# rgl-epfl/large-steps-pytorch

Measured on AMD Instinct MI355X. Metric: from_differential_solves_per_sec, higher is better.
Workload: dtype f32; 1 GPU; cfg4_plane1m: 1000x1000 plane, V=1000000, nnz(M)=6992002, M=I+50*L_uniform, u=M v, k=3, factor once (not timed), re-solve timed; method=nested-dissection, device=AMD Radeon Graphics

## Files before the change

### include/largesteps_hip.h

```cpp
#ifndef LARGESTEPS_HIP_H
#define LARGESTEPS_HIP_H

#include <stddef.h>
#include <stdint.h>

#ifdef __cplusplus
extern "C" {
#endif

#define LS_VERSION 110

#define LS_OK 0
#define LS_E_INVALID (-1)
#define LS_E_INDEX (-2)
#define LS_E_WORKSPACE (-3)
#define LS_E_OVERFLOW (-4)
#define LS_E_STATE (-5)
#define LS_E_NOT_CONVERGED (-6)

#define LS_LAPLACIAN_UNIFORM 0
#define LS_LAPLACIAN_COT 1

int ls_version(void);
const char* ls_last_error(void);
// ... 97 lines not shown
    const int64_t* h_nodes;
    const int32_t* h_perm;
    const int32_t* h_ppos;
    int64_t n_bnd;
    const int32_t* h_push_ptr;
    const int32_t* h_push_tgt;
    int64_t n_front;
    const float* d_finv;
    const float* d_wf;
    const float* d_wb;
    const float* d_u4;
    const float* d_d4;
    const float* d_tri;
    const int32_t* d_sp_ptr;
    const void* d_sp_ent;
    int64_t n_sp_ptr, n_sp_ent;
    int32_t shard_rank, shard_count;
    int32_t tier_waves;
} ls_direct_arrays;
int ls_direct_create(const ls_direct_arrays* arrays, int device, void* stream, ls_direct** out);
int ls_direct_pick_tree(int64_t V, int* leaf_size, int* arity);
int ls_direct_tier_lds_bytes(int levels, int arity, const int32_t* h_s, const int32_t* h_b, const int32_t* h_own_start, int tier_levels,
                             int sparse_leaves, int waves, size_t* h_bytes);
int ls_direct_factor(const int32_t* d_rowptr, const int32_t* d_col, const float* d_val, int64_t V, int64_t nnz,
                     const float* d_positions, int leaf_size, int arity, int tier_levels, int sparse_leaves, int shard_rank,
                     int shard_count, int device, void* stream, ls_direct** out);
typedef struct ls_direct_options {
    int32_t struct_bytes;
    int32_t leaf_size, arity, tier_levels, sparse_leaves, shard_rank, shard_count;
    int32_t ordering;
    int32_t tier_waves;
} ls_direct_options;
int ls_direct_options_default(ls_direct_options* opt);
int ls_direct_factor_ex(const int32_t* d_rowptr, const int32_t* d_col, const float* d_val, int64_t V, int64_t nnz,
                        const float* d_positions, const ls_direct_options* opt, int device, void* stream, ls_direct** out);
int ls_direct_factor_refactorable(const int32_t* d_rowptr, const int32_t* d_col, const float* d_val, int64_t V, int64_t nnz,
                                  const float* d_positions, const ls_direct_options* opt, int device, void* stream, ls_direct** out);
int ls_direct_refactor(ls_direct* d, const int32_t* d_rowptr, const int32_t* d_col, const float* d_val, int64_t V, int64_t nnz,
                       void* stream);
int ls_direct_refactorable(const ls_direct* d, int* h_yes, size_t* h_retained_device_bytes);
int ls_release_scratch(int device);
int ls_direct_shape(const ls_direct* d, int* h_levels, int* h_arity, int* h_tier_levels, int* h_tier_workgroups,
                    int64_t* h_words_up, int64_t* h_words_down, int64_t* h_n_bnd);
int ls_direct_level_words(const ls_direct* d, int cap, int64_t* h_up, int64_t* h_down);
int ls_direct_level_rows(const ls_direct* d, int cap, int64_t* h_rows, int64_t* h_bnd);
int ls_direct_level_index_bytes(const ls_direct* d, int cap, int64_t* h_up, int64_t* h_down);
int ls_direct_tier_balance(const ls_direct* d, double* h_words4);
int ls_direct_launch_profile(const ls_direct* d, int cap, int* h_n, double* h_ms, int64_t* h_words, int32_t* h_level_lo,
                             int32_t* h_level_hi, int32_t* h_sweep);
int ls_direct_plan_quality(const ls_direct* d, int* h_ordering, double* h_words_per_vertex, double* h_spread, double* h_words_other);
int ls_direct_factor_seconds(const ls_direct* d, double* h_s3);
int ls_csr_is_symmetric(const int32_t* d_rowptr, const int32_t* d_col, const float* d_val, int64_t V, int64_t nnz, float tol,
                        int* h_symmetric, int device, void* stream);
int ls_direct_destroy(ls_direct* d);
int ls_direct_solve(ls_direct* d, const float* b, float* x, int k, void* stream);
int ls_direct_solve_part(ls_direct* d, const float* b, float* x, int k, int part, float* exchange, void* stream);
int ls_direct_shard_info(const ls_direct* d, int* h_rank, int* h_count, int* h_cut_level, int64_t* h_exchange_floats_per_column,
                         unsigned char* h_owned_rows);
int ls_direct_exchange_region(ls_direct* d, int k, float** h_region, int64_t* h_floats);

typedef struct ls_dist ls_dist;
int ls_dist_unique_id(void* h_id128);
int ls_dist_create(const void* h_id128, int rank, int world, int device, ls_dist** out);
int ls_dist_destroy(ls_dist* c);
int ls_dist_allreduce_sum(ls_dist* c, float* d_buf, int64_t n, void* stream);
int ls_dist_info(const ls_dist* c, int* h_rank, int* h_world);
int ls_dist_direct_solve(ls_dist* c, ls_direct* d, const float* b, float* x, int k, void* stream);
int ls_direct_set(ls_direct* d, const char* name, int value);
int ls_direct_info(const ls_direct* d, int64_t* h_factor_entries, int* h_launches, double* h_ms3);

int ls_remove_duplicates_workspace_bytes(int64_t V, size_t* h_bytes);
int ls_remove_duplicates(const float* verts, int64_t V, const void* faces, int idx_bytes, int64_t F, float* unique_verts,
                         int64_t* inverse, int64_t* new_faces, int64_t* h_n_unique, void* workspace, size_t ws_bytes, int device,
                         void* stream);

int ls_csr_transpose_workspace_bytes(int64_t V, int64_t nnz, size_t* h_bytes);
int ls_csr_transpose(const int32_t* rowptr, const int32_t* col, const float* val, int64_t V, int64_t nnz, int32_t* t_rowptr,
                     int32_t* t_col, float* t_val, void* workspace, size_t ws_bytes, int device, void* stream);
int ls_corner_ranks_workspace_bytes(int64_t F, int64_t V, size_t* h_bytes);
int ls_corner_ranks(const void* faces, int idx_bytes, int64_t F, int64_t V, int32_t* vptr, int32_t* cpos, void* workspace,
                    size_t ws_bytes, int device, void* stream);

int ls_normals_workspace_bytes(int64_t F, int64_t V, size_t* h_bytes);
int ls_face_normals(const float* verts, const void* faces, int idx_bytes, int64_t F, int64_t V, float* fn, int device, void* stream);
int ls_face_normals_backward(const float* verts, const void* faces, int idx_bytes, int64_t F, int64_t V, const int32_t* vptr,
                             const int32_t* cpos, const float* g_fn, float* grad_verts, void* workspace, size_t ws_bytes,
                             int device, void* stream);
int ls_vertex_normals(const float* verts, const void* faces, int idx_bytes, int64_t F, int64_t V, const int32_t* vptr,
                      const int32_t* cpos, const float* fn, float* out, float* raw, float* norms, void* workspace,
                      size_t ws_bytes, int device, void* stream);
int ls_vertex_normals_backward(const float* verts, const void* faces, int idx_bytes, int64_t F, int64_t V, const int32_t* vptr,
// ... 189 lines not shown
```

### large-steps-pytorch_amd/csrc/direct.hip

```cpp
#include "common.h"
#include <vector>
#include <chrono>
#include <algorithm>
#include <atomic>
#include <string.h>
#include <memory>
#include <mutex>

namespace ls {

struct alignas(64) Tile {
    int store;
    int row0, s, b, own_start, bnd_off, front_off;
    int leaf;
    int pfront_off, cix;
    int forward;
    int arity;
    long long finv_off, w_off;
};

static_assert(sizeof(Tile) == 64, "Tile layout");
__device__ __forceinline__ Tile load_tile(const Tile* __restrict__ tiles, int idx) {
    const int lane = threadIdx.x & 63;
    const int w = lane < 16 ? reinterpret_cast<const int*>(tiles)[(size_t)idx * 16 + lane] : 0;
// ... 705 lines not shown
    const float *finv = nullptr, *wf = nullptr, *wb = nullptr;
    const float *u4 = nullptr, *d4 = nullptr;
    const float* tri = nullptr;
    const int* sp_ptr = nullptr;
    const SpEnt* sp_ent = nullptr;
    float* braw = nullptr;
    float *bp = nullptr, *slots = nullptr, *xb = nullptr;
    int upper_lo = 0;
    int tier_root = 0, tier_phases = 0, tier_wgs = 0, tier_region = 0, tier_vec = 0, tier_tri = 0, tier_waves = TIER_WAVES;
    TierItem* d_items = nullptr;
    int* pull = nullptr;
    int64_t pull_base = 0;
    TierWG* d_wgs = nullptr;
    hipEvent_t busy = nullptr;
    hipStream_t last_stream = nullptr;
    bool used = false;
    std::vector<std::pair<void*, size_t>> tables;
    ls::RefactorState* refac = nullptr;
    bool factored = true;
    int shard_rank = 0, shard_count = 1, cut = 0;
    int64_t exch_f0 = 0, exch_f1 = 0;
    std::vector<unsigned char> owned_rows;
    bool nt_levels = false, nt_tier = false, nt_rule[2] = {false, false};
    double factor_s[3] = {0, 0, 0};
    double plan_q[4] = {0, 0, 0, 0};
    std::vector<LevelPlan> plan;
    int64_t factor_entries = 0, words_up = 0, words_down = 0;
    int profile = 0;
    std::vector<hipEvent_t> ev;
    struct LaunchMeta { int lo, hi, sweep; };
    std::vector<hipEvent_t> lev;
    std::vector<LaunchMeta> lmeta;
    std::vector<double> launch_ms;
    std::vector<int64_t> lvl_up, lvl_down;
    std::vector<int64_t> lvl_rows, lvl_bnd;
    std::vector<int64_t> lvl_idx_up, lvl_idx_down;
    double tier_balance[4] = {0, 0, 0, 0};
    double prof_ms[3] = {0, 0, 0};
#ifdef LS_TIER_STAMPS
    long long* stamps = nullptr;
#endif
};

static int pick_nw(int len, int target) {
    int nw = 1;
    while (nw < 16 && len > nw * target) nw *= 2;
// ... 191 lines not shown
    memset(nd.data(), 0, nd.size() * sizeof(NodeD));
    const int root = levels - tier_levels;
    for (int lv = root; lv < levels; ++lv)
        for (int64_t i = level_off[lv]; i < level_off[lv + 1]; ++i) {
            NodeD& q = nd[(size_t)i];
            q.s = s[i]; q.b = b[i]; q.own_start = own_start[i];
            const bool sparse = sparse_leaves && lv == levels - 1 && q.s >= 1;
            q.flags = (lv + 1 >= levels ? NODE_LEAF : 0) | (sparse ? NODE_SPARSE : NODE_QUAD);
        }
    std::vector<TierItem> items;
    std::vector<TierWG> wgs;
    int vec = 0, tri = 0;
    const size_t region = plan_tier(nd, level_off, levels, arity, root, 0, level_off[root + 1] - level_off[root], items, wgs, vec, tri, waves);
    return region ? ((region + 3) & ~(size_t)3) * sizeof(float) * waves : 0;
}

bool direct_tier_fits(int levels, int arity, const int* s, const int* b, const int* own_start, int tier_levels, bool sparse_leaves, int waves) {
    if (tier_levels <= 0) return true;
    if (tier_levels > levels || tier_levels > TIER_MAX_H) return false;
    const size_t bytes = direct_tier_lds(levels, arity, s, b, own_start, tier_levels, sparse_leaves, waves);
    return bytes && bytes <= (size_t)(waves == TIER_WAVES_FULL ? TIER_LDS_FULL : TIER_LDS);
}

extern "C" int ls_direct_tier_lds_bytes(int levels, int arity, const int32_t* h_s, const int32_t* h_b, const int32_t* h_own_start, int tier_levels,
                                        int sparse_leaves, int waves, size_t* h_bytes) {
    LS_REQUIRE(h_s && h_b && h_own_start && h_bytes && levels >= 1 && levels <= 30 && (arity == 2 || arity == 4 || arity == 8) &&
               tier_levels >= 1 && tier_levels <= levels && tier_levels <= TIER_MAX_H && (waves == TIER_WAVES || waves == TIER_WAVES_WIDE || waves == TIER_WAVES_FULL),
               LS_E_INVALID, "ls_direct_tier_lds_bytes: bad argument (1 <= tier_levels <= min(levels, %d); waves 4, 8 or 16)", TIER_MAX_H);
    *h_bytes = direct_tier_lds(levels, arity, h_s, h_b, h_own_start, tier_levels, sparse_leaves != 0, waves);
    return LS_OK;
}

bool direct_tier_full16(int64_t V, int arity, int levels, int tier_levels, int shard_count, int tier_waves) {
    if (tier_waves == TIER_WAVES_FULL) return tier_levels >= 2;
    if (tier_waves == TIER_WAVES || tier_waves == TIER_WAVES_WIDE) return false;
    return shard_count <= 1 && arity == 4 && levels >= 8 && V >= 800000 && tier_levels == levels - 4 && tier_levels <= TIER_MAX_H;
}


namespace {
struct CreatePlan {
    int levels = 0, arity = 0, cut = 0;
    int64_t sub_lo = 0, sub_hi = 1;
    std::vector<int64_t> level_off;
    std::vector<NodeD> nd;
    std::vector<int> parent;
// ... 93 lines not shown
    if (T.cut > root) { set_error("ls_direct_create: %d ranks need a cut below the tier's root level (tree too small)", d->shard_count); return LS_E_INVALID; }
    const int64_t span = T.span(T.cut, root), q_lo = T.sub_lo * span, q_hi = T.sub_hi * span;
    size_t region = 0;
    auto take_if_fits = [&](int waves, int budget) {
        std::vector<TierItem> items;
        std::vector<TierWG> wgs;
        int vec = 0, tri = 0;
        const size_t r = plan_tier(T.nd, T.level_off, levels, T.arity, root, q_lo, q_hi, items, wgs, vec, tri, waves);
        if (!r || ((r + 3) & ~(size_t)3) * sizeof(float) * waves > (size_t)budget) return;
        T.items.swap(items); T.wgs.swap(wgs); d->tier_vec = vec; d->tier_tri = tri; region = r; d->tier_waves = waves;
    };
    if (H <= TIER_MAX_H && direct_tier_full16(d->V, T.arity, levels, H, d->shard_count, tier_waves > 0 ? tier_waves : env.tier_waves.value_or(0)))
        take_if_fits(TIER_WAVES_FULL, TIER_LDS_FULL);
    if (!region) {
        region = H <= TIER_MAX_H ? plan_tier(T.nd, T.level_off, levels, T.arity, root, q_lo, q_hi, T.items, T.wgs, d->tier_vec, d->tier_tri) : 0;
        if (!region || region * sizeof(float) * TIER_WAVES > TIER_LDS) {
            set_error("ls_direct_create: a tier of %d levels does not fit the kernel (LDS per wave: %zu floats)", H, region);
            return LS_E_WORKSPACE;
        }
        if (H >= 2 && (int)T.wgs.size() <= 768 && (tier_waves > 0 ? tier_waves : env.tier_waves.value_or(TIER_WAVES_WIDE)) == TIER_WAVES_WIDE)
            take_if_fits(TIER_WAVES_WIDE, TIER_LDS_WIDE);
    }
    d->tier_root = root; d->tier_phases = H; d->tier_wgs = (int)T.wgs.size(); d->tier_region = (int)((region + 3) & ~(size_t)3);
    d->pull_base = T.nd[T.level_off[root]].front_off;
    T.pull.assign((size_t)std::max<int64_t>(0, T.nd[T.level_off[levels - 1]].front_off - d->pull_base) * T.arity, -1);
    for (int lv = root + 1; lv < levels; ++lv)
        for (int64_t i = T.level_off[lv]; i < T.level_off[lv + 1]; ++i) {
            const NodeD& n = T.nd[i];
            for (int k = 0; k < n.b; ++k) T.pull[(size_t)(n.pfront_off - d->pull_base + h_ppos[n.bnd_off + k]) * T.arity + n.cix] = n.bnd_off + k;
        }
    return LS_OK;
}

size_t plan_level(CreatePlan& T, int lv, int long_up, const NdEnv& env, int kmax, LevelPlan& p) {
    std::vector<Tile>& tiles = T.tiles;
    int64_t a0 = T.level_off[lv], a1 = T.level_off[lv + 1];
    if (lv >= T.cut) { const int64_t span = T.span(T.cut, lv); a0 = T.level_off[lv] + T.sub_lo * span; a1 = T.level_off[lv] + T.sub_hi * span; }
    auto tile_of = [&](int64_t i, int r, int forward) {
        const NodeD& n = T.nd[i];
        Tile t;
        t.store = 0; t.row0 = r; t.s = n.s; t.b = n.b; t.own_start = n.own_start; t.bnd_off = n.bnd_off; t.front_off = n.front_off;
        t.leaf = lv + 1 >= T.levels; t.pfront_off = n.pfront_off; t.cix = n.cix;
        t.forward = forward; t.arity = T.arity; t.finv_off = n.finv_off; t.w_off = n.w_off;
        return t;
    };
    int red_up = 0, red_down = 0;
// ... 266 lines not shown
    if (d->busy) (void)hipEventDestroy(d->busy);
    if (!d->tables.empty()) (void)hipDeviceSynchronize();
    for (const auto& t : d->tables)
        if (!ls::pool_give(d->device, t.first, t.second)) (void)hipFree(t.first);
    ls::refactor_state_free(d->refac);
    for (hipEvent_t e : d->ev) (void)hipEventDestroy(e);
#ifdef LS_TIER_STAMPS
    if (d->stamps) (void)hipFree(d->stamps);
#endif
    for (hipEvent_t e : d->lev) (void)hipEventDestroy(e);
    delete d;
    return LS_OK;
}

template <int K>
static int direct_solve_k(ls_direct* d, const float* b, float* x, hipStream_t st, int part, float* exchange) {
    const int top = d->tier_root - 1;
    TierArgs ta;
    ta.items = d->d_items; ta.wgs = d->d_wgs; ta.perm = d->perm; ta.mask = d->mask; ta.ppos = d->ppos;
    ta.pull = d->pull ? d->pull - (size_t)d->pull_base * d->arity : nullptr; ta.push_ptr = d->push_ptr; ta.push_tgt = d->push_tgt; ta.u4 = d->u4; ta.d4 = d->d4; ta.tri = d->tri;
    ta.sp_ptr = d->sp_ptr; ta.sp_ent = d->sp_ent; ta.bprime = d->bp; ta.braw = d->braw; ta.slots = d->slots; ta.xb = d->xb;
    ta.arity = d->arity; ta.phases = d->tier_phases; ta.region_floats = d->tier_region; ta.vec_floats = d->tier_vec;
    ta.upper_lo = d->upper_lo; ta.upper_hi = (int)d->V;
#ifdef LS_TIER_STAMPS
    const size_t stamp_n = (size_t)d->tier_wgs * d->tier_waves * TIER_STAMP_SLOTS;
    if (d->profile == 2 && !d->stamps && stamp_n) LS_HIP(hipMalloc((void**)&d->stamps, 2 * stamp_n * sizeof(long long)));
    if (d->profile == 2 && d->stamps) LS_HIP(hipMemsetAsync(d->stamps, 0, 2 * stamp_n * sizeof(long long), st));
    ta.stamps = d->profile == 2 ? d->stamps : nullptr;
#endif
    const size_t tier_lds = (size_t)d->tier_region * d->tier_waves * sizeof(float);
    const bool nt_tier = d->nt_tier && d->tier_waves != TIER_WAVES_WIDE, nt = d->nt_levels;
    int n_mark = 0;
    auto mark = [&](int lo, int hi, int sweep) -> hipError_t {
        if (d->profile != 3) return hipSuccess;
        while ((int)d->lev.size() <= n_mark + 1) { hipEvent_t e; const hipError_t r = hipEventCreate(&e); if (r != hipSuccess) return r; d->lev.push_back(e); }
        if ((int)d->lmeta.size() <= n_mark) d->lmeta.resize((size_t)n_mark + 1);
        d->lmeta[(size_t)n_mark] = {lo, hi, sweep};
        return hipEventRecord(d->lev[(size_t)n_mark++], st);
    };
    auto mark_end = [&]() -> hipError_t {
        if (d->profile != 3) return hipSuccess;
        hipError_t r = hipEventRecord(d->lev[(size_t)n_mark], st);
        if (r == hipSuccess) r = hipStreamSynchronize(st);
        d->launch_ms.assign((size_t)n_mark, 0.0);
        d->lmeta.resize((size_t)n_mark);
        for (int i = 0; i < n_mark && r == hipSuccess; ++i) { float ms = 0; r = hipEventElapsedTime(&ms, d->lev[(size_t)i], d->lev[(size_t)i + 1]); d->launch_ms[(size_t)i] = ms; }
        return r;
    };
    const size_t exch_off = (size_t)d->exch_f0 * d->arity * K, exch_n = (size_t)(d->exch_f1 - d->exch_f0) * d->arity * K;
    if (part != 1) {
    if (d->profile) LS_HIP(hipEventRecord(d->ev[0], st));
    if (part == 0 && exch_n) LS_HIP(hipMemsetAsync(d->slots + exch_off, 0, exch_n * sizeof(float), st));
    if (d->tier_wgs) {
// ... 139 lines not shown
    if (h_cut_level) *h_cut_level = d->cut;
    if (h_exchange_floats_per_column) *h_exchange_floats_per_column = (d->exch_f1 - d->exch_f0) * d->arity;
    if (h_owned_rows) { if (d->owned_rows.empty()) memset(h_owned_rows, 1, (size_t)d->V); else memcpy(h_owned_rows, d->owned_rows.data(), (size_t)d->V); }
    return LS_OK;
}

extern "C" int ls_direct_set(ls_direct* d, const char* name, int value) {
    LS_REQUIRE(d && name, LS_E_INVALID, "ls_direct_set: bad argument");
    if (!strcmp(name, "profile")) {
        DeviceGuard g(d->device);
        LS_HIP(g.err);
#ifndef LS_TIER_STAMPS
        LS_REQUIRE(value != 2, LS_E_INVALID, "ls_direct_set: profile 2 (per-wave clock stamps of the tier kernels) exists in the experiments build only (tools/build_variant.sh stamps -DLS_TIER_STAMPS)");
#endif
        d->profile = value < 0 ? 0 : std::min(value, 3);
        while (d->profile && d->ev.size() < 4) { hipEvent_t e; LS_HIP(hipEventCreate(&e)); d->ev.push_back(e); }
        return LS_OK;
    }
    if (!strcmp(name, "nt")) {
        d->nt_levels = value < 0 ? d->nt_rule[0] : value != 0;
        d->nt_tier = value < 0 ? d->nt_rule[1] : value != 0;
        return LS_OK;
    }
    set_error("ls_direct_set: unknown option '%s'", name);
    return LS_E_INVALID;
}

int ls_direct_adopt(ls_direct* d, std::vector<std::pair<void*, size_t>> owned, const double* seconds3, const double* quality4, ls::RefactorState* refac) {
    d->tables.insert(d->tables.end(), owned.begin(), owned.end());
    d->refac = refac;
    for (int i = 0; i < 3; ++i) d->factor_s[i] = seconds3[i];
    for (int i = 0; i < 4; ++i) d->plan_q[i] = quality4[i];
    return LS_OK;
}

extern "C" int ls_direct_refactor(ls_direct* d, const int32_t* d_rowptr, const int32_t* d_col, const float* d_val, int64_t V, int64_t nnz,
                                  void* stream) {
    LS_REQUIRE(d && d_rowptr && d_col && d_val && V > 0 && nnz > 0, LS_E_INVALID, "ls_direct_refactor: bad argument");
    LS_REQUIRE(d->refac, LS_E_STATE, "ls_direct_refactor: %s", d->shard_count > 1 ? "a sharded handle cannot refactor"
                                                                                  : "the handle was not made by ls_direct_factor_refactorable");
    DeviceGuard g(d->device);
    LS_HIP(g.err);
    hipStream_t st = (hipStream_t)stream;
    hipStreamCaptureStatus cap = hipStreamCaptureStatusNone;
    if (st) (void)hipStreamIsCapturing(st, &cap);
    LS_REQUIRE(cap == hipStreamCaptureStatusNone, LS_E_STATE, "ls_direct_refactor: not capturable (it synchronises the stream)");
// ... 14 lines not shown

extern "C" int ls_direct_plan_quality(const ls_direct* d, int* h_ordering, double* h_words_per_vertex, double* h_spread, double* h_words_other) {
    LS_REQUIRE(d, LS_E_INVALID, "ls_direct_plan_quality: bad argument");
    if (h_ordering) *h_ordering = (int)d->plan_q[0];
    if (h_words_per_vertex) *h_words_per_vertex = d->plan_q[1];
    if (h_spread) *h_spread = d->plan_q[2];
    if (h_words_other) *h_words_other = d->plan_q[3];
    return LS_OK;
}

extern "C" int ls_direct_shape(const ls_direct* d, int* h_levels, int* h_arity, int* h_tier_levels, int* h_tier_workgroups,
                               int64_t* h_words_up, int64_t* h_words_down, int64_t* h_n_bnd) {
    LS_REQUIRE(d, LS_E_INVALID, "ls_direct_shape: bad argument");
    if (h_words_up) *h_words_up = d->words_up;
    if (h_words_down) *h_words_down = d->words_down;
    if (h_n_bnd) *h_n_bnd = d->n_bnd;
    if (h_levels) *h_levels = d->levels;
    if (h_arity) *h_arity = d->arity;
    if (h_tier_levels) *h_tier_levels = d->tier_phases;
    if (h_tier_workgroups) *h_tier_workgroups = d->tier_wgs;
    return LS_OK;
}

extern "C" int ls_direct_factor_seconds(const ls_direct* d, double* h_s3) {
    LS_REQUIRE(d && h_s3, LS_E_INVALID, "ls_direct_factor_seconds: bad argument");
    for (int i = 0; i < 3; ++i) h_s3[i] = d->factor_s[i];
    return LS_OK;
}

extern "C" int ls_direct_level_words(const ls_direct* d, int cap, int64_t* h_up, int64_t* h_down) {
    LS_REQUIRE(d && cap >= 0, LS_E_INVALID, "ls_direct_level_words: bad argument");
    for (int lv = 0; lv < cap && lv < d->levels; ++lv) {
        if (h_up) h_up[lv] = lv < (int)d->lvl_up.size() ? d->lvl_up[(size_t)lv] : 0;
        if (h_down) h_down[lv] = lv < (int)d->lvl_down.size() ? d->lvl_down[(size_t)lv] : 0;
    }
    return LS_OK;
}

extern "C" int ls_direct_level_rows(const ls_direct* d, int cap, int64_t* h_rows, int64_t* h_bnd) {
    LS_REQUIRE(d && cap >= 0, LS_E_INVALID, "ls_direct_level_rows: bad argument");
    for (int lv = 0; lv < cap && lv < d->levels; ++lv) {
        if (h_rows) h_rows[lv] = lv < (int)d->lvl_rows.size() ? d->lvl_rows[(size_t)lv] : 0;
        if (h_bnd) h_bnd[lv] = lv < (int)d->lvl_bnd.size() ? d->lvl_bnd[(size_t)lv] : 0;
    }
    return LS_OK;
}
// ... 65 lines not shown
```

### large-steps-pytorch_amd/csrc/nd_tier.h

```cpp
#pragma once

namespace ls {

constexpr int TIER_MAX_H = 6;
constexpr int TIER_WAVES = 4;
constexpr int TIER_WAVES_WIDE = 8;
constexpr int TIER_WAVES_FULL = 16;
constexpr int TIER_LDS_FULL = 160 * 1024;
constexpr int TIER_LDS = 150 * 1024;
constexpr int TIER_LDS_WIDE = 80 * 1024;
constexpr int LEVEL_LDS = 150 * 1024;
constexpr int LDS_OPTIN = 160 * 1024;
constexpr int TIER_TRI4 = 9;
constexpr int TIER_SPE = 4;

enum : int { NODE_LEAF = 1, NODE_SPARSE = 2, NODE_QUAD = 4, NODE_UPC = 8 };

struct SpEnt { float val; int idx; };

struct NodeD {
    int s, b, own_start, bnd_off, front_off, pfront_off, cix, flags;
    long long finv_off, w_off;
    int spb_off, sps_off;
};
// ... 16 lines not shown
};
static_assert(sizeof(TierWG) == 128, "TierWG layout (read as 32 dwords)");

struct TierArgs {
    const TierItem* items;
    const TierWG* wgs;
    const int* perm;
    const unsigned char* mask;
    const int* ppos;
    const int* pull;
    const int* push_ptr;
    const int* push_tgt;
    const float* u4;
    const float* d4;
    const float* tri;
    const int* sp_ptr;
    const SpEnt* sp_ent;
    float* bprime;
    int upper_lo, upper_hi;
    float* braw;
    float* slots;
    float* xb;
    int arity, phases, region_floats, vec_floats;
#ifdef LS_TIER_STAMPS
    long long* stamps;
#endif
};

constexpr int TIER_STAMP_SLOTS = 32;
#ifdef LS_TIER_STAMPS
#define LS_STAMP(slot) do { if (a.stamps && lane == 0) stamp_base[(slot)] = (long long)wall_clock64(); } while (0)
#define LS_STAMP_VAL(slot, v) do { if (a.stamps && lane == 0) stamp_base[(slot)] = (long long)(v); } while (0)
#else
#define LS_STAMP(slot) do { } while (0)
#define LS_STAMP_VAL(slot, v) do { } while (0)
#endif

constexpr int ITEM_DWORDS = 24;
__device__ __forceinline__ int rec_load(const TierItem* items, int k, int lane) {
    return lane < ITEM_DWORDS ? reinterpret_cast<const int*>(items)[(size_t)k * ITEM_DWORDS + lane] : 0;
}
__device__ __forceinline__ int rl(int v, int i) { return __builtin_amdgcn_readlane(v, i); }
__device__ __forceinline__ TierItem rec_unpack(int r) {
    TierItem t;
    t.s = rl(r, 0); t.b = rl(r, 1); t.own_start = rl(r, 2); t.bnd_off = rl(r, 3); t.front_off = rl(r, 4); t.pfront_off = rl(r, 5);
    t.cix = rl(r, 6); t.flags = rl(r, 7);
// ... 42 lines not shown
#pragma unroll
    for (int c0 = 0; c0 < A; c0 += G) {
        int pg[G];
        float r[G][K];
#pragma unroll
        for (int c = 0; c < G; ++c) pg[c] = pl[c0 + c];
        pull_request<K, G>(a, pg, r);
        pull_sum<K, G>(pg, r, v);
    }
}
template <int K>
__device__ __forceinline__ void pull_compact(const TierArgs& a, size_t f, float (&v)[K]) {
#pragma unroll
    for (int q = 0; q < K; ++q) v[q] = 0.0f;
    if (a.arity == 4) pull_compact_n<K, 4>(a, f, v);
    else if (a.arity == 8) pull_compact_n<K, 8>(a, f, v);
    else pull_compact_n<K, 2>(a, f, v);
}

__device__ __forceinline__ void pull_indices(const TierArgs& a, size_t f, bool on, int (&pl)[4]) {
#pragma unroll
    for (int c = 0; c < 4; ++c) pl[c] = on ? a.pull[f * 4 + c] : -1;
}

struct LeafIdx {
    int g, p0, p1, pp;
};
template <int K>
struct LeafDat {
    float4 t[TIER_TRI4];
    float v[K];
    float xv[K];
    SpEnt e[TIER_SPE];
};

template <bool UP>
__device__ __forceinline__ void leaf_idx(const TierArgs& a, const TierItem& n, int lane, LeafIdx& ix) {
    ix.g = lane < n.s ? a.perm[n.own_start + lane] : 0;
    if (UP) {
        const bool r = lane < n.b;
        ix.p0 = r ? a.sp_ptr[n.spb_off + lane] : 0;
        ix.p1 = r ? a.sp_ptr[n.spb_off + lane + 1] : 0;
        ix.pp = r ? a.ppos[n.bnd_off + lane] : 0;
    } else {
        const bool r = lane < n.s;
        ix.p0 = r ? a.sp_ptr[n.sps_off + lane] : 0;
// ... 190 lines not shown

template <int K>
__device__ __forceinline__ void leaf_down_vec(const TierItem& n, const float (&t)[K], float* region, int tri_floats) {
    const int lane = threadIdx.x & 63;
    float4 w = make_float4(0.f, 0.f, 0.f, 0.f);
    if (lane < n.s) { w.x = t[0]; if (K > 1) w.y = t[K > 1 ? 1 : 0]; if (K > 2) w.z = t[K > 2 ? 2 : 0]; if (K > 3) w.w = t[K > 3 ? 3 : 0]; }
    reinterpret_cast<float4*>(region + tri_floats)[lane] = w;
}

template <int K>
__device__ __forceinline__ void leaf_down_tail(const TierItem& n, const LeafIdx& ix, const float (&yj)[K], float* __restrict__ x_out,
                                               float* region, int tri_floats) {
    const int lane = threadIdx.x & 63, s = n.s;
    float z[K];
    tri_matvec<K>(region, region + tri_floats, s, lane, z);
    if (lane < s) {
#pragma unroll
        for (int q = 0; q < K; ++q) x_out[(size_t)ix.g * K + q] = yj[q] - z[q];
    }
    wave_lds_sync();
}

template <int K, bool UP, int W, bool NT>
__device__ __forceinline__ void leaf_phase(const TierArgs& a, int k0, int k1, const float* __restrict__ b_in, float* __restrict__ x_out,
                                           float* region, int tri_floats, long long* stamp_base) {
    const int lane = threadIdx.x & 63;
    int leaf_no = 0;
    (void)leaf_no; (void)stamp_base;
    if (k0 >= k1) return;
    constexpr int S = W;
    TierItem it = rec_unpack(rec_load(a.items, k0, lane));
    int rec_n = k0 + S < k1 ? rec_load(a.items, k0 + S, lane) : 0;
    LeafIdx ix;
    leaf_idx<UP>(a, it, lane, ix);
    for (int k = k0; k < k1; k += S) {
        float v[K];
        SpEnt e[TIER_SPE];
        float t[K];
        {
            LeafDat<K> d;
            leaf_dat<K, UP, NT>(a, it, ix, b_in, lane, d);
            if (!UP) leaf_down_head<K>(a, it, ix, d.xv, d.e, region, t);
            tri_stage<K>(d, it.s, lane, region);
#pragma unroll
            for (int q = 0; q < K; ++q) v[q] = d.v[q];
#pragma unroll
            for (int u = 0; u < TIER_SPE; ++u) e[u] = d.e[u];
        }
        if (!UP) leaf_down_vec<K>(it, t, region, tri_floats);
        wave_lds_sync();
        const bool more = k + S < k1;
        TierItem it_n = it;
        LeafIdx ix_n = ix;
        if (more) { it_n = rec_unpack(rec_n); leaf_idx<UP>(a, it_n, lane, ix_n); }
        rec_n = k + 2 * S < k1 ? rec_load(a.items, k + 2 * S, lane) : 0;
        if (UP) leaf_up_compute<K>(a, it, ix, v, e, region, tri_floats);
        else leaf_down_tail<K>(it, ix, v, x_out, region, tri_floats);
        if (leaf_no < 8) LS_STAMP(16 + leaf_no);
        ++leaf_no;
        it = it_n; ix = ix_n;
    }
}

#ifndef LS_TIER_Q
#define LS_TIER_Q 4
#endif
constexpr int TIER_Q = LS_TIER_Q;

template <bool NT>
__device__ __forceinline__ void tier_prefetch(const float4* __restrict__ col, size_t rows, int q0, int q1, float4 (&cur)[TIER_Q]) {
#pragma unroll
    for (int e = 0; e < TIER_Q; ++e) cur[e] = (q0 + e < q1) ? ld_stream4<NT>(col + (size_t)(q0 + e) * rows) : make_float4(0.f, 0.f, 0.f, 0.f);
}

__device__ __forceinline__ void tier_mv16(float v16, const float4& a, const float4& b, const float4& c, const float4& d, int n, f32x4& acc) {
    acc = mv_step<0>(v16, a.x, acc); acc = mv_step<1>(v16, a.y, acc); acc = mv_step<2>(v16, a.z, acc); acc = mv_step<3>(v16, a.w, acc);
    if (n > 1) { acc = mv_step<4>(v16, b.x, acc); acc = mv_step<5>(v16, b.y, acc); acc = mv_step<6>(v16, b.z, acc); acc = mv_step<7>(v16, b.w, acc); }
    if (n > 2) { acc = mv_step<8>(v16, c.x, acc); acc = mv_step<9>(v16, c.y, acc); acc = mv_step<10>(v16, c.z, acc); acc = mv_step<11>(v16, c.w, acc); }
    if (n > 3) { acc = mv_step<12>(v16, d.x, acc); acc = mv_step<13>(v16, d.y, acc); acc = mv_step<14>(v16, d.z, acc); acc = mv_step<15>(v16, d.w, acc); }
}

__device__ __forceinline__ void tier_mv_batch(const float* sv4, int base, int q, int q1, const float4 (&c)[TIER_Q], f32x4& acc) {
    const int lane = threadIdx.x & 63;
    const float4 z = make_float4(0.f, 0.f, 0.f, 0.f);
// ... 253 lines not shown
            push_down<K>(a.push_tgt, p0, p1, a.xb, v);
        }
    }
    wave_lds_sync();
}

template <int K, bool UP, int W, bool NT>
__global__ __launch_bounds__(64 * W, W >= 16 ? 1 : 4) void k_nd_tier(TierArgs a, const float* __restrict__ b_in, float* __restrict__ x_out,
                                                              int tri_floats) {
    extern __shared__ __attribute__((aligned(16))) float sm[];
    const int wave = __builtin_amdgcn_readfirstlane(threadIdx.x >> 6), lane = threadIdx.x & 63;
    float* region = sm + (size_t)wave * a.region_floats;
    for (int i = lane; 4 * i < a.region_floats; i += 64) reinterpret_cast<float4*>(region)[i] = make_float4(0.f, 0.f, 0.f, 0.f);
    wave_lds_sync();
    const int n_wg = (int)gridDim.x;
    const int sub = __builtin_expect((n_wg & 7) == 0, 1) ? (int)(blockIdx.x & 7) * (n_wg >> 3) + (int)(blockIdx.x >> 3) : (int)blockIdx.x;
#ifdef LS_TIER_STAMPS
    long long* stamp_base = a.stamps ? a.stamps + ((size_t)sub * W + wave) * TIER_STAMP_SLOTS : nullptr;
#else
    long long* stamp_base = nullptr;
#endif
    LS_STAMP(0);
    const int hdr = lane < 32 ? reinterpret_cast<const int*>(a.wgs + sub)[lane] : 0;
    const int obase = UP ? 0 : TIER_MAX_H + 1;
    const unsigned split = (unsigned)rl(hdr, UP ? 14 : 15), leafy = (unsigned)rl(hdr, UP ? 16 : 17);
    if (UP) {
        const int n_dense = rl(hdr, 18);
        for (int r = threadIdx.x; r < n_dense; r += blockDim.x) {
            int o = r, start = 0;
#pragma unroll
            for (int t = 0; t < TIER_MAX_H; ++t) {
                const int cnt = rl(hdr, 20 + 2 * t + 1);
                const bool here = o >= 0 && o < cnt;
                start = here ? rl(hdr, 20 + 2 * t) + o : start;
                o = here ? -1 : o - cnt;
            }
            const size_t g = (size_t)a.perm[start];
#pragma unroll
            for (int q = 0; q < K; ++q) a.braw[(size_t)start * K + q] = b_in[g * K + q];
        }
        for (int r = a.upper_lo + blockIdx.x * blockDim.x + threadIdx.x; r < a.upper_hi; r += gridDim.x * blockDim.x) {
            const size_t g = (size_t)a.perm[r];
#pragma unroll
            for (int q = 0; q < K; ++q) a.braw[(size_t)r * K + q] = b_in[g * K + q];
        }
    }
    LS_STAMP(1);
    DensePre<K> pre;
#pragma unroll
    for (int e = 0; e < TIER_Q; ++e) pre.cur[e] = make_float4(0.f, 0.f, 0.f, 0.f);
#pragma unroll
    for (int q = 0; q < K; ++q) pre.v[q] = 0.0f;
    pre.idx = 0; pre.fw0 = 1; pre.fw1 = 0;
#pragma unroll
    for (int c = 0; c < 4; ++c) { pre.plo[c] = -1; pre.plb[c] = -1; }
    TierItem it_pre = rec_unpack(0);
    bool pre_valid = false;
    for (int ph = 0; ph < a.phases; ++ph) {
        const int i0 = rl(hdr, obase + ph), i1 = rl(hdr, obase + ph + 1);
        int rec_nx = 0;
        bool has_nx = false;
        if (ph + 1 < a.phases && !((leafy >> (ph + 1)) & 1u)) {
            const int j0 = rl(hdr, obase + ph + 1) + wave;
            has_nx = j0 < rl(hdr, obase + ph + 2);
            if (has_nx) rec_nx = rec_load(a.items, j0, lane);
        }
        if ((leafy >> ph) & 1u) {
            leaf_phase<K, UP, W, NT>(a, i0 + wave, i1, b_in, x_out, region, tri_floats, stamp_base);
        } else {
            int rec = (!pre_valid && i0 + wave < i1) ? rec_load(a.items, i0 + wave, lane) : 0;
            int head_k = -1, head_idx = 0, head_p0 = 0, head_p1 = 0, head_flags = 0;
            for (int k = i0 + wave; k < i1; k += W) {
                const int rec_next = k + W < i1 ? rec_load(a.items, k + W, lane) : 0;
                const bool first = k == i0 + wave && pre_valid;
                const TierItem it = first ? it_pre : rec_unpack(rec);
                rec = rec_next;
                float* pbuf = region + a.vec_floats + ((k - i0) / W) * 256;
                if (!first) { if (UP) node_up_pre<K, NT>(a, it, pre); else node_down_pre<K, NT>(a, it, pre); }
                if (UP) node_up<K, NT>(a, it, pre, b_in, region, pbuf);
                else node_down<K, NT>(a, it, pre, x_out, region, pbuf);
                if (it.nparts > 1 && it.part == 0) {
                    head_k = k; head_idx = pre.idx; head_p0 = pre.plo[0]; head_p1 = pre.plo[1]; head_flags = it.flags;
                }
            }
            if ((split >> ph) & 1u) {
                const int rec_head = head_k >= 0 ? rec_load(a.items, head_k, lane) : 0;
                int head_tg[4];
#pragma unroll
                for (int c = 0; c < 4; ++c) head_tg[c] = (!UP && head_k >= 0 && head_p0 + c < head_p1 && !(head_flags & NODE_LEAF)) ? a.push_tgt[head_p0 + c] : -1;
                __syncthreads();
                for (int k = i0 + wave; k < i1; k += W) {
                    const bool mine = k == head_k;
                    const TierItem it = rec_unpack(mine ? rec_head : rec_load(a.items, k, lane));
                    if (it.nparts == 1 || it.part != 0) continue;
                    float acc[K];
#pragma unroll
                    for (int q = 0; q < K; ++q) acc[q] = 0.0f;
                    for (int p = 0; p < it.nparts; ++p) {
                        const int kp = k + p - i0;
                        const float* pb = sm + (size_t)(kp % W) * a.region_floats + a.vec_floats + (kp / W) * 256;
#pragma unroll
                        for (int q = 0; q < K; ++q) acc[q] += pb[lane * 4 + q];
                    }
                    if (UP) {
                        const int i = it.row0 + lane;
                        const int pp = mine ? head_idx : ((i < it.b && it.pfront_off >= 0 && !(it.flags & NODE_UPC)) ? a.ppos[it.bnd_off + i] : 0);
                        node_up_finish<K>(a, it, i, pp, acc);
                    } else if (mine) {
                        node_down_store<K>(a, it, head_idx, head_p0, head_p1, head_tg, x_out, acc);
                    }
                    else node_down_finish<K>(a, it, x_out, acc);
                }
            }
        }
        if (ph < 6) { LS_STAMP(2 + 2 * ph); LS_STAMP_VAL(24 + ph, (i1 - i0 - wave + W - 1) / W); }
        pre_valid = has_nx;
        it_pre = rec_unpack(rec_nx);
        if (pre_valid) {
            if (UP) node_up_pre<K, NT>(a, it_pre, pre); else node_down_pre<K, NT>(a, it_pre, pre);
        } else {
#pragma unroll
            for (int e = 0; e < TIER_Q; ++e) pre.cur[e] = make_float4(0.f, 0.f, 0.f, 0.f);
#pragma unroll
            for (int q = 0; q < K; ++q) pre.v[q] = 0.0f;
            pre.idx = 0; pre.fw0 = 1; pre.fw1 = 0;
#pragma unroll
            for (int c = 0; c < 4; ++c) { pre.plo[c] = -1; pre.plb[c] = -1; }
        }
        __syncthreads();
        if (ph < 6) LS_STAMP(3 + 2 * ph);
    }
}

}
```

### large-steps-pytorch_amd/largesteps/_native.py

```python
import ctypes
import os
import threading
import weakref

import torch

_HERE = os.path.dirname(os.path.abspath(__file__))
_LIB_PATH = os.environ.get("LARGESTEPS_HIP_LIB", os.path.join(_HERE, "..", "lib", "liblargesteps_hip.so"))

LS_E_INVALID, LS_E_INDEX, LS_E_WORKSPACE, LS_E_OVERFLOW, LS_E_STATE, LS_E_NOT_CONVERGED = -1, -2, -3, -4, -5, -6

_lib = None
_lib_lock = threading.Lock()

c_void_p, c_int, c_i64, c_float, c_double, c_size_t = (ctypes.c_void_p, ctypes.c_int, ctypes.c_int64, ctypes.c_float,
                                                        ctypes.c_double, ctypes.c_size_t)


class SolveInfo(ctypes.Structure):
    _fields_ = [("iterations", ctypes.c_int32), ("converged", ctypes.c_int32),
                ("rnorm", ctypes.c_double * 4), ("bnorm", ctypes.c_double * 4)]


class DirectOptions(ctypes.Structure):
# ... 89 lines not shown
    "ls_iso_count": (c_int, [c_void_p, c_i64, c_i64, c_i64, c_float, c_void_p, c_size_t, c_void_p, c_int, c_void_p]),
    "ls_iso_fill": (c_int, [c_void_p, c_i64, c_i64, c_i64, c_float, c_void_p, c_void_p, c_void_p, c_size_t, c_i64, c_i64, c_void_p,
                            c_void_p, c_void_p, c_int, c_void_p]),
    "ls_iso_backward": (c_int, [c_void_p, c_i64, c_i64, c_i64, c_float, c_void_p, c_void_p, c_void_p, c_size_t, c_i64, c_void_p,
                                c_void_p, c_int, c_void_p]),
    "ls_mesh_ray_backward": (c_int, [c_void_p, c_void_p, c_void_p, c_i64, c_void_p, c_void_p, c_void_p, c_void_p, c_void_p, c_void_p, c_void_p,
                                     c_void_p, c_void_p, c_void_p, c_size_t, c_void_p]),
    "ls_sample_workspace_bytes": (c_int, [c_i64, c_i64, ctypes.POINTER(c_size_t)]),
    "ls_sample_surface": (c_int, [c_void_p, c_void_p, c_int, c_i64, c_i64, c_i64, ctypes.c_uint64, ctypes.c_uint32, ctypes.c_uint64, c_void_p,
                                  c_void_p, c_void_p, c_void_p, c_size_t, c_int, c_void_p]),
    "ls_sample_surface_backward": (c_int, [c_void_p, c_int, c_i64, c_i64, c_i64, c_void_p, c_void_p, c_void_p, c_void_p, c_void_p, c_void_p,
                                           c_void_p, c_size_t, c_int, c_void_p]),
    "ls_shard_plan_create": (c_int, [c_i64, c_void_p, c_void_p, c_void_p, c_int, c_int, c_int, ctypes.POINTER(c_void_p)]),
    "ls_shard_plan_destroy": (c_int, [c_void_p]),
    "ls_shard_plan_info": (c_int, [c_void_p] + [ctypes.POINTER(c_i64)] * 5 + [ctypes.POINTER(c_int)] * 2 + [ctypes.POINTER(c_i64)]),
    "ls_shard_plan_arrays": (c_int, [c_void_p] + [c_void_p] * 8),
    "ls_shard_layer_sizes": (c_int, [c_i64, c_void_p, c_void_p, c_i64, c_i64, c_int, c_void_p]),
    "ls_patch_plan_create": (c_int, [c_i64, c_void_p, c_void_p, c_void_p, c_void_p, c_int, c_int, c_int, c_int, c_int, ctypes.POINTER(c_void_p)]),
    "ls_patch_plan_destroy": (c_int, [c_void_p]),
    "ls_patch_plan_info": (c_int, [c_void_p] + [ctypes.POINTER(c_int)] * 5 + [ctypes.POINTER(c_i64)] * 3 + [ctypes.POINTER(ctypes.c_double)]),
    "ls_patch_plan_arrays": (c_int, [c_void_p, c_void_p, c_void_p, c_void_p, c_void_p, c_void_p]),
    "ls_direct_level_words": (c_int, [c_void_p, c_int, c_void_p, c_void_p]),
    "ls_direct_tier_lds_bytes": (c_int, [c_int, c_int, c_void_p, c_void_p, c_void_p, c_int, c_int, c_int, ctypes.POINTER(c_size_t)]),
    "ls_direct_level_index_bytes": (c_int, [c_void_p, c_int, c_void_p, c_void_p]),
    "ls_direct_tier_balance": (c_int, [c_void_p, ctypes.POINTER(c_double * 4)]),
    "ls_direct_level_rows": (c_int, [c_void_p, c_int, c_void_p, c_void_p]),
    "ls_direct_exchange_region": (c_int, [c_void_p, c_int, ctypes.POINTER(c_void_p), ctypes.POINTER(c_i64)]),
    "ls_dist_unique_id": (c_int, [c_void_p]),
    "ls_dist_create": (c_int, [c_void_p, c_int, c_int, c_int, ctypes.POINTER(c_void_p)]),
    "ls_dist_destroy": (c_int, [c_void_p]),
    "ls_dist_allreduce_sum": (c_int, [c_void_p, c_void_p, c_i64, c_void_p]),
    "ls_dist_info": (c_int, [c_void_p, ctypes.POINTER(c_int), ctypes.POINTER(c_int)]),
    "ls_dist_direct_solve": (c_int, [c_void_p, c_void_p, c_void_p, c_void_p, c_int, c_void_p]),
    "ls_direct_launch_profile": (c_int, [c_void_p, c_int, c_void_p, c_void_p, c_void_p, c_void_p, c_void_p, c_void_p]),
    "ls_direct_factor": (c_int, [c_void_p, c_void_p, c_void_p, c_i64, c_i64, c_void_p, c_int, c_int, c_int, c_int, c_int, c_int, c_int,
                                 c_void_p, ctypes.POINTER(c_void_p)]),
    "ls_direct_factor_ex": (c_int, [c_void_p, c_void_p, c_void_p, c_i64, c_i64, c_void_p, c_void_p, c_int, c_void_p, ctypes.POINTER(c_void_p)]),
    "ls_direct_options_default": (c_int, [c_void_p]),
    "ls_direct_factor_refactorable": (c_int, [c_void_p, c_void_p, c_void_p, c_i64, c_i64, c_void_p, c_void_p, c_int, c_void_p,
                                              ctypes.POINTER(c_void_p)]),
    "ls_direct_refactor": (c_int, [c_void_p, c_void_p, c_void_p, c_void_p, c_i64, c_i64, c_void_p]),
    "ls_direct_refactorable": (c_int, [c_void_p, ctypes.POINTER(c_int), ctypes.POINTER(c_size_t)]),
    "ls_direct_solve_part": (c_int, [c_void_p, c_void_p, c_void_p, c_int, c_int, c_void_p, c_void_p]),
    "ls_direct_shard_info": (c_int, [c_void_p, ctypes.POINTER(c_int), ctypes.POINTER(c_int), ctypes.POINTER(c_int), ctypes.POINTER(c_i64),
                                     c_void_p]),
    "ls_direct_shape": (c_int, [c_void_p, ctypes.POINTER(c_int), ctypes.POINTER(c_int), ctypes.POINTER(c_int), ctypes.POINTER(c_int),
# ... 352 lines not shown
```

### large-steps-pytorch_amd/largesteps/solvers.py

```python
import ctypes
import os
import types
import warnings

import numpy as np
import torch
from torch.autograd import Function

from . import _native

_KMAX = 4


class Solver:
    generation = 0

    def __init__(self, M):
        pass

    def solve(self, b, backward=False):
        raise NotImplementedError()


class PCGSolver(Solver):
# ... 208 lines not shown
        if rc:
            _native.check(rc)

    def refactor(self, csr):
        if not self._h.value:
            raise RuntimeError("this solver was closed")
        with torch.cuda.device(self.device):
            rc = _native.lib().ls_direct_refactor(self._h, _native.ptr(csr.rowptr), _native.ptr(csr.col), _native.ptr(csr.val), csr.V, csr.nnz,
                                                  _native.stream_of(self.device))
        self.factored = rc == 0 or (self.factored and (rc == _native.LS_E_STATE or "the factor is unchanged" in _native.last_error()))
        _native.check(rc)

    def set_option(self, name, value):
        _native.check(_native.lib().ls_direct_set(self._h, name.encode(), int(value)))

    def info(self):
        fe, nl = ctypes.c_int64(0), ctypes.c_int(0)
        ms = (ctypes.c_double * 3)()
        _native.check(_native.lib().ls_direct_info(self._h, ctypes.byref(fe), ctypes.byref(nl), ms))
        lv, ar, th, tw = ctypes.c_int(0), ctypes.c_int(0), ctypes.c_int(0), ctypes.c_int(0)
        wu, wd, nb = ctypes.c_int64(0), ctypes.c_int64(0), ctypes.c_int64(0)
        _native.check(_native.lib().ls_direct_shape(self._h, ctypes.byref(lv), ctypes.byref(ar), ctypes.byref(th), ctypes.byref(tw),
                                                    ctypes.byref(wu), ctypes.byref(wd), ctypes.byref(nb)))
        return dict(factor_entries=fe.value, launches=nl.value, up_ms=ms[0], down_ms=ms[1], mid_ms=ms[2], levels=lv.value, arity=ar.value,
                    tier_levels=th.value, tier_workgroups=tw.value, words_up=wu.value, words_down=wd.value, n_bnd=nb.value)


    def level_words(self):
        n = self.info()["levels"]
        up, down = (ctypes.c_int64 * n)(), (ctypes.c_int64 * n)()
        _native.check(_native.lib().ls_direct_level_words(self._h, n, up, down))
        return list(up), list(down)

    def level_rows(self):
        n = self.info()["levels"]
        rows, bnd = (ctypes.c_int64 * n)(), (ctypes.c_int64 * n)()
        _native.check(_native.lib().ls_direct_level_rows(self._h, n, rows, bnd))
        return list(rows), list(bnd)

    def level_index_bytes(self):
        n = self.info()["levels"]
        up, down = (ctypes.c_int64 * n)(), (ctypes.c_int64 * n)()
        _native.check(_native.lib().ls_direct_level_index_bytes(self._h, n, up, down))
        return list(up), list(down)

    def tier_balance(self):
        w = (ctypes.c_double * 4)()
        _native.check(_native.lib().ls_direct_tier_balance(self._h, ctypes.byref(w)))
# ... 268 lines not shown
```

Baseline: 5310 solves/s.

## Deal tier leaf items to waves dynamically via LDS ticket counter

Replaces the static strided assignment of leaf items to waves in the tier kernel with a dynamic work-stealing scheme. Each wave takes its next item from a workgroup-scope atomic counter held in a small extra LDS slot, using double-buffered counters across phases. It is enabled by default only when the extra LDS does not reduce occupancy. The aim is to balance uneven leaf costs across waves, at the price of an atomic per item, an added barrier, and the possibility that workgroup occupancy or the prefetch pattern changes.

```diff
diff --git a/include/largesteps_hip.h b/include/largesteps_hip.h
--- a/include/largesteps_hip.h
+++ b/include/largesteps_hip.h
@@ -143,6 +143,7 @@
 int ls_direct_pick_tree(int64_t V, int* leaf_size, int* arity);
 int ls_direct_tier_lds_bytes(int levels, int arity, const int32_t* h_s, const int32_t* h_b, const int32_t* h_own_start, int tier_levels,
                              int sparse_leaves, int waves, size_t* h_bytes);
+int ls_direct_tier_deal_fits(size_t tier_lds_bytes, int waves, int* h_yes);
 int ls_direct_factor(const int32_t* d_rowptr, const int32_t* d_col, const float* d_val, int64_t V, int64_t nnz,
                      const float* d_positions, int leaf_size, int arity, int tier_levels, int sparse_leaves, int shard_rank,
                      int shard_count, int device, void* stream, ls_direct** out);
@@ -188,6 +189,7 @@
 int ls_dist_info(const ls_dist* c, int* h_rank, int* h_world);
 int ls_dist_direct_solve(ls_dist* c, ls_direct* d, const float* b, float* x, int k, void* stream);
 int ls_direct_set(ls_direct* d, const char* name, int value);
+int ls_direct_tier_deal(const ls_direct* d, int* h_on, int* h_fits);
 int ls_direct_info(const ls_direct* d, int64_t* h_factor_entries, int* h_launches, double* h_ms3);
 
 int ls_remove_duplicates_workspace_bytes(int64_t V, size_t* h_bytes);
diff --git a/large-steps-pytorch_amd/csrc/direct.hip b/large-steps-pytorch_amd/csrc/direct.hip
--- a/large-steps-pytorch_amd/csrc/direct.hip
+++ b/large-steps-pytorch_amd/csrc/direct.hip
@@ -751,6 +751,7 @@
     int64_t exch_f0 = 0, exch_f1 = 0;
     std::vector<unsigned char> owned_rows;
     bool nt_levels = false, nt_tier = false, nt_rule[2] = {false, false};
+    bool tier_deal = false, tier_deal_fits = false;
     double factor_s[3] = {0, 0, 0};
     double plan_q[4] = {0, 0, 0, 0};
     std::vector<LevelPlan> plan;
@@ -988,6 +989,19 @@
     return bytes && bytes <= (size_t)(waves == TIER_WAVES_FULL ? TIER_LDS_FULL : TIER_LDS);
 }
 
+bool direct_tier_deal_fits(size_t tier_lds_bytes, int waves) {
+    if (!tier_lds_bytes || tier_lds_bytes + TIER_DEAL_LDS > (size_t)LDS_OPTIN) return false;
+    const size_t by_waves = (size_t)(TIER_WAVES_FULL / waves);
+    return std::min(by_waves, (size_t)LDS_OPTIN / (tier_lds_bytes + TIER_DEAL_LDS)) == std::min(by_waves, (size_t)LDS_OPTIN / tier_lds_bytes);
+}
+
+extern "C" int ls_direct_tier_deal_fits(size_t tier_lds_bytes, int waves, int* h_yes) {
+    LS_REQUIRE(h_yes && (waves == TIER_WAVES || waves == TIER_WAVES_WIDE || waves == TIER_WAVES_FULL), LS_E_INVALID,
+               "ls_direct_tier_deal_fits: bad argument (waves 4, 8 or 16)");
+    *h_yes = direct_tier_deal_fits(tier_lds_bytes, waves) ? 1 : 0;
+    return LS_OK;
+}
+
 extern "C" int ls_direct_tier_lds_bytes(int levels, int arity, const int32_t* h_s, const int32_t* h_b, const int32_t* h_own_start, int tier_levels,
                                         int sparse_leaves, int waves, size_t* h_bytes) {
     LS_REQUIRE(h_s && h_b && h_own_start && h_bytes && levels >= 1 && levels <= 30 && (arity == 2 || arity == 4 || arity == 8) &&
@@ -1127,6 +1141,7 @@
             take_if_fits(TIER_WAVES_WIDE, TIER_LDS_WIDE);
     }
     d->tier_root = root; d->tier_phases = H; d->tier_wgs = (int)T.wgs.size(); d->tier_region = (int)((region + 3) & ~(size_t)3);
+    d->tier_deal = d->tier_deal_fits = direct_tier_deal_fits((size_t)d->tier_region * d->tier_waves * sizeof(float), d->tier_waves);
     d->pull_base = T.nd[T.level_off[root]].front_off;
     T.pull.assign((size_t)std::max<int64_t>(0, T.nd[T.level_off[levels - 1]].front_off - d->pull_base) * T.arity, -1);
     for (int lv = root + 1; lv < levels; ++lv)
@@ -1439,13 +1454,14 @@
     ta.sp_ptr = d->sp_ptr; ta.sp_ent = d->sp_ent; ta.bprime = d->bp; ta.braw = d->braw; ta.slots = d->slots; ta.xb = d->xb;
     ta.arity = d->arity; ta.phases = d->tier_phases; ta.region_floats = d->tier_region; ta.vec_floats = d->tier_vec;
     ta.upper_lo = d->upper_lo; ta.upper_hi = (int)d->V;
+    ta.deal = d->tier_deal ? 1 : 0;
 #ifdef LS_TIER_STAMPS
     const size_t stamp_n = (size_t)d->tier_wgs * d->tier_waves * TIER_STAMP_SLOTS;
     if (d->profile == 2 && !d->stamps && stamp_n) LS_HIP(hipMalloc((void**)&d->stamps, 2 * stamp_n * sizeof(long long)));
     if (d->profile == 2 && d->stamps) LS_HIP(hipMemsetAsync(d->stamps, 0, 2 * stamp_n * sizeof(long long), st));
     ta.stamps = d->profile == 2 ? d->stamps : nullptr;
 #endif
-    const size_t tier_lds = (size_t)d->tier_region * d->tier_waves * sizeof(float);
+    const size_t tier_lds = (size_t)d->tier_region * d->tier_waves * sizeof(float) + (d->tier_deal ? TIER_DEAL_LDS : 0);
     const bool nt_tier = d->nt_tier && d->tier_waves != TIER_WAVES_WIDE, nt = d->nt_levels;
     int n_mark = 0;
     auto mark = [&](int lo, int hi, int sweep) -> hipError_t {
@@ -1631,6 +1647,12 @@
         d->nt_tier = value < 0 ? d->nt_rule[1] : value != 0;
         return LS_OK;
     }
+    if (!strcmp(name, "tier_deal")) {
+        LS_REQUIRE(value == 0 || value == 1, LS_E_INVALID, "ls_direct_set: tier_deal is 0 or 1");
+        LS_REQUIRE(!value || d->tier_deal_fits, LS_E_INVALID, "ls_direct_set: tier_deal = 1 needs %d bytes of LDS behind the tier's regions; this handle has none to spare", TIER_DEAL_LDS);
+        d->tier_deal = value != 0;
+        return LS_OK;
+    }
     set_error("ls_direct_set: unknown option '%s'", name);
     return LS_E_INVALID;
 }
@@ -1691,6 +1713,13 @@
     return LS_OK;
 }
 
+extern "C" int ls_direct_tier_deal(const ls_direct* d, int* h_on, int* h_fits) {
+    LS_REQUIRE(d, LS_E_INVALID, "ls_direct_tier_deal: bad argument");
+    if (h_on) *h_on = d->tier_deal ? 1 : 0;
+    if (h_fits) *h_fits = d->tier_deal_fits ? 1 : 0;
+    return LS_OK;
+}
+
 extern "C" int ls_direct_factor_seconds(const ls_direct* d, double* h_s3) {
     LS_REQUIRE(d && h_s3, LS_E_INVALID, "ls_direct_factor_seconds: bad argument");
     for (int i = 0; i < 3; ++i) h_s3[i] = d->factor_s[i];
diff --git a/large-steps-pytorch_amd/csrc/nd_tier.h b/large-steps-pytorch_amd/csrc/nd_tier.h
--- a/large-steps-pytorch_amd/csrc/nd_tier.h
+++ b/large-steps-pytorch_amd/csrc/nd_tier.h
@@ -62,6 +62,7 @@
     float* slots;
     float* xb;
     int arity, phases, region_floats, vec_floats;
+    int deal;
 #ifdef LS_TIER_STAMPS
     long long* stamps;
 #endif
@@ -150,6 +151,14 @@
 #pragma unroll
     for (int c = 0; c < 4; ++c) pl[c] = on ? a.pull[f * 4 + c] : -1;
 }
+
+constexpr int TIER_DEAL_LDS = 16;
+__device__ __forceinline__ int ticket_take(int* ctr, int lane) {
+    int t = 0;
+    if (lane == 0) t = (int)__builtin_amdgcn_atomic_inc32(reinterpret_cast<unsigned*>(ctr), 0xffffffffu, __ATOMIC_RELAXED, "workgroup");
+    return t;
+}
+__device__ __forceinline__ int ticket_of(int raw) { return __builtin_amdgcn_readfirstlane(raw); }
 
 struct LeafIdx {
     int g, p0, p1, pp;
@@ -386,12 +395,12 @@
 }
 
 template <int K, bool UP, int W, bool NT>
-__device__ __forceinline__ void leaf_phase(const TierArgs& a, int k0, int k1, const float* __restrict__ b_in, float* __restrict__ x_out,
-                                           float* region, int tri_floats, long long* stamp_base) {
+__device__ __forceinline__ int leaf_phase(const TierArgs& a, int k0, int k1, const float* __restrict__ b_in, float* __restrict__ x_out,
+                                          float* region, int tri_floats, long long* stamp_base) {
     const int lane = threadIdx.x & 63;
     int leaf_no = 0;
-    (void)leaf_no; (void)stamp_base;
-    if (k0 >= k1) return;
+    (void)stamp_base;
+    if (k0 >= k1) return 0;
     constexpr int S = W;
     TierItem it = rec_unpack(rec_load(a.items, k0, lane));
     int rec_n = k0 + S < k1 ? rec_load(a.items, k0 + S, lane) : 0;
@@ -424,6 +433,51 @@
         ++leaf_no;
         it = it_n; ix = ix_n;
     }
+    return leaf_no;
+}
+
+template <int K, bool UP, int W, bool NT>
+__device__ __forceinline__ int leaf_phase_dealt(const TierArgs& a, int i0, int i1, int wave, int* ctr, const float* __restrict__ b_in,
+                                                float* __restrict__ x_out, float* region, int tri_floats, long long* stamp_base) {
+    const int lane = threadIdx.x & 63;
+    int leaf_no = 0;
+    (void)stamp_base;
+    if (i0 + wave >= i1) return 0;
+    TierItem it = rec_unpack(rec_load(a.items, i0 + wave, lane));
+    LeafIdx ix;
+    leaf_idx<UP>(a, it, lane, ix);
+    for (;;) {
+        float v[K];
+        SpEnt e[TIER_SPE];
+        float t[K];
+        const int raw = ticket_take(ctr, lane);
+        int kn, rec_n;
+        {
+            LeafDat<K> d;
+            leaf_dat<K, UP, NT>(a, it, ix, b_in, lane, d);
+            kn = i0 + ticket_of(raw);
+            rec_n = kn < i1 ? rec_load(a.items, kn, lane) : 0;
+            if (!UP) leaf_down_head<K>(a, it, ix, d.xv, d.e, region, t);
+            tri_stage<K>(d, it.s, lane, region);
+#pragma unroll
+            for (int q = 0; q < K; ++q) v[q] = d.v[q];
+#pragma unroll
+            for (int u = 0; u < TIER_SPE; ++u) e[u] = d.e[u];
+        }
+        if (!UP) leaf_down_vec<K>(it, t, region, tri_floats);
+        wave_lds_sync();
+        const bool more = kn < i1;
+        TierItem it_n = it;
+        LeafIdx ix_n = ix;
+        if (more) { it_n = rec_unpack(rec_n); leaf_idx<UP>(a, it_n, lane, ix_n); }
+        if (UP) leaf_up_compute<K>(a, it, ix, v, e, region, tri_floats);
+        else leaf_down_tail<K>(it, ix, v, x_out, region, tri_floats);
+        if (leaf_no < 8) LS_STAMP(16 + leaf_no);
+        ++leaf_no;
+        if (!more) break;
+        it = it_n; ix = ix_n;
+    }
+    return leaf_no;
 }
 
 #ifndef LS_TIER_Q
@@ -723,8 +777,11 @@
 #endif
     LS_STAMP(0);
     const int hdr = lane < 32 ? reinterpret_cast<const int*>(a.wgs + sub)[lane] : 0;
+    int* const deal_ctr = a.deal ? reinterpret_cast<int*>(sm + (size_t)W * a.region_floats) : nullptr;
+    if (deal_ctr && threadIdx.x == 0) { deal_ctr[0] = W; deal_ctr[1] = W; }
     const int obase = UP ? 0 : TIER_MAX_H + 1;
     const unsigned split = (unsigned)rl(hdr, UP ? 14 : 15), leafy = (unsigned)rl(hdr, UP ? 16 : 17);
+    if (deal_ctr && (leafy & 1u)) __syncthreads();
     if (UP) {
         const int n_dense = rl(hdr, 18);
         for (int r = threadIdx.x; r < n_dense; r += blockDim.x) {
@@ -766,8 +823,13 @@
             has_nx = j0 < rl(hdr, obase + ph + 2);
             if (has_nx) rec_nx = rec_load(a.items, j0, lane);
         }
+        int* const ctr = deal_ctr ? deal_ctr + (ph & 1) : nullptr;
+        if (deal_ctr && ph > 0 && threadIdx.x == 0) deal_ctr[(ph + 1) & 1] = W;
+        int n_ran = 0;
+        (void)n_ran;
         if ((leafy >> ph) & 1u) {
-            leaf_phase<K, UP, W, NT>(a, i0 + wave, i1, b_in, x_out, region, tri_floats, stamp_base);
+            if (ctr) n_ran = leaf_phase_dealt<K, UP, W, NT>(a, i0, i1, wave, ctr, b_in, x_out, region, tri_floats, stamp_base);
+            else n_ran = leaf_phase<K, UP, W, NT>(a, i0 + wave, i1, b_in, x_out, region, tri_floats, stamp_base);
         } else {
             int rec = (!pre_valid && i0 + wave < i1) ? rec_load(a.items, i0 + wave, lane) : 0;
             int head_k = -1, head_idx = 0, head_p0 = 0, head_p1 = 0, head_flags = 0;
@@ -783,6 +845,7 @@
                 if (it.nparts > 1 && it.part == 0) {
                     head_k = k; head_idx = pre.idx; head_p0 = pre.plo[0]; head_p1 = pre.plo[1]; head_flags = it.flags;
                 }
+                ++n_ran;
             }
             if ((split >> ph) & 1u) {
                 const int rec_head = head_k >= 0 ? rec_load(a.items, head_k, lane) : 0;
@@ -814,7 +877,7 @@
                 }
             }
         }
-        if (ph < 6) { LS_STAMP(2 + 2 * ph); LS_STAMP_VAL(24 + ph, (i1 - i0 - wave + W - 1) / W); }
+        if (ph < 6) { LS_STAMP(2 + 2 * ph); LS_STAMP_VAL(24 + ph, n_ran); }
         pre_valid = has_nx;
         it_pre = rec_unpack(rec_nx);
         if (pre_valid) {
diff --git a/large-steps-pytorch_amd/largesteps/_native.py b/large-steps-pytorch_amd/largesteps/_native.py
--- a/large-steps-pytorch_amd/largesteps/_native.py
+++ b/large-steps-pytorch_amd/largesteps/_native.py
@@ -135,6 +135,8 @@
     "ls_patch_plan_arrays": (c_int, [c_void_p, c_void_p, c_void_p, c_void_p, c_void_p, c_void_p]),
     "ls_direct_level_words": (c_int, [c_void_p, c_int, c_void_p, c_void_p]),
     "ls_direct_tier_lds_bytes": (c_int, [c_int, c_int, c_void_p, c_void_p, c_void_p, c_int, c_int, c_int, ctypes.POINTER(c_size_t)]),
+    "ls_direct_tier_deal_fits": (c_int, [c_size_t, c_int, ctypes.POINTER(c_int)]),
+    "ls_direct_tier_deal": (c_int, [c_void_p, ctypes.POINTER(c_int), ctypes.POINTER(c_int)]),
     "ls_direct_level_index_bytes": (c_int, [c_void_p, c_int, c_void_p, c_void_p]),
     "ls_direct_tier_balance": (c_int, [c_void_p, ctypes.POINTER(c_double * 4)]),
     "ls_direct_level_rows": (c_int, [c_void_p, c_int, c_void_p, c_void_p]),
diff --git a/large-steps-pytorch_amd/largesteps/solvers.py b/large-steps-pytorch_amd/largesteps/solvers.py
--- a/large-steps-pytorch_amd/largesteps/solvers.py
+++ b/large-steps-pytorch_amd/largesteps/solvers.py
@@ -254,8 +254,11 @@
         wu, wd, nb = ctypes.c_int64(0), ctypes.c_int64(0), ctypes.c_int64(0)
         _native.check(_native.lib().ls_direct_shape(self._h, ctypes.byref(lv), ctypes.byref(ar), ctypes.byref(th), ctypes.byref(tw),
                                                     ctypes.byref(wu), ctypes.byref(wd), ctypes.byref(nb)))
+        deal = ctypes.c_int(0)
+        _native.check(_native.lib().ls_direct_tier_deal(self._h, ctypes.byref(deal), None))
         return dict(factor_entries=fe.value, launches=nl.value, up_ms=ms[0], down_ms=ms[1], mid_ms=ms[2], levels=lv.value, arity=ar.value,
-                    tier_levels=th.value, tier_workgroups=tw.value, words_up=wu.value, words_down=wd.value, n_bnd=nb.value)
+                    tier_levels=th.value, tier_workgroups=tw.value, words_up=wu.value, words_down=wd.value, n_bnd=nb.value,
+                    tier_deal=deal.value)
 
 
     def level_words(self):
```

Measured after the change: 5284 solves/s. About the same (-0.5%).
